# laomao0/BIN

Hardware: AMD Instinct MI355X
Metric: interpolated frames/sec at 1280x720 (higher is better)
Workload: dtype f16x3 (fp16 hi+lo pairs = 22-bit significands, 3 MFMA products, f32 accumulate; fp32-class: 1e-6 vs the fp32 reference); 1 GPU; Adobe240 test_blur 1280x720 inference, batch=1 per GPU (6-frame window padded to 768x1344 by the test.py rule), window-sharded; precision=f16x3, streams=1, pipelined_steps=False, four_call_schedule=False, parity=max-abs <= 2e-5 (f16x3) vs the fp32 reference (tests/)

## Files before the change

### bin_amd/csrc/binhip_conv_x3.hip

```cpp
#include "binhip_conv_common.h"
constexpr int X3_R = 2, X3_WN = 8;

template <int KS, int R, int WN, int NTAP = KS * KS>
struct X3Cfg {
    static constexpr int PAD = KS / 2;
    static constexpr int TH = R * WN;
    static constexpr int PH = TH + KS - 1;
    static constexpr int PW = 32 + KS - 1;
    static constexpr int PP = (PH * PW * 2 + 63) / 64;
    static constexpr int WP = NTAP;
    static constexpr int NW = WN;
    static constexpr int PATCH_BYTES = PP * 1024;
    static constexpr int WBUF_BYTES = 2 * WP * 1024;
    static constexpr int LDS_BYTES = 2 * PATCH_BYTES + 2 * WBUF_BYTES;
    static constexpr int NPJ = (PP + NW - 1) / NW;
    static constexpr int NWJ = (2 * WP + NW - 1) / NW;
    static_assert((KS == 3 ? 2 : 1) * LDS_BYTES <= 160 * 1024, "LDS budget");
};
constexpr int X3_FOLD_TAPS = 20;
template <int KS, int R, int WN, int EPI>
using X3CfgOf = X3Cfg<KS, R, WN, EPI == BINHIP_EPI_SUBPIX_FOLD ? X3_FOLD_TAPS : KS * KS>;

template <class C>
__device__ __forceinline__ void x3_issue_patch(const ConvKArgs& a, char* smem, int c, int pl, int buf, int wave,
                                               const unsigned* voff, const ConvTile& t) {
    __amdgpu_buffer_rsrc_t rs = patch_plane_grouped(a, c, pl, t);
    char* lds = smem + buf * C::PATCH_BYTES;
#pragma unroll
    for (int j = 0; j < C::NPJ; ++j) {
        const int i = wave + C::NW * j;
        if ((C::PP % C::NW == 0) || (i < C::PP))
            __builtin_amdgcn_raw_ptr_buffer_load_lds(rs, (lds_void_t*)(lds + i * 1024), 16, voff[j], 0, 0, 0);
    }
}

template <class C>
__device__ __forceinline__ void x3_issue_weights(const ConvKArgs& a, char* smem, int c, int buf, int wave, int lane, int z) {
    const long long woff = ((long long)z * a.nchunks + c) * (C::WP * 32 * 16);
    __amdgpu_buffer_rsrc_t wh = __builtin_amdgcn_make_buffer_rsrc((void*)(a.w_hi + woff), 0, C::WP * 1024, 0x00020000);
    __amdgpu_buffer_rsrc_t wl = __builtin_amdgcn_make_buffer_rsrc((void*)(a.w_lo + woff), 0, C::WP * 1024, 0x00020000);
    char* lds = smem + 2 * C::PATCH_BYTES + buf * C::WBUF_BYTES;
#pragma unroll
    for (int j = 0; j < C::NWJ; ++j) {
        const int i = wave + C::NW * j;
        if (((2 * C::WP) % C::NW == 0) || (i < 2 * C::WP)) {
            const bool lo = i >= C::WP;
            const int t = lo ? i - C::WP : i;
            __builtin_amdgcn_raw_ptr_buffer_load_lds(lo ? wl : wh, (lds_void_t*)(lds + i * 1024), 16,
                                                     (unsigned)(lane * 16), t * 1024, 0, 0);
        }
    }
}

template <class C, int KS, int R, bool HI>
__device__ __forceinline__ void x3_compute(const char* pb, const char* wb, int a_lane_off, int b_lane_off, floatx16 (&acc)[R]) {
    constexpr int NTAP = KS * KS;
    half8 B[2][R + KS - 1];
    half8 Ah[2], Al[2];
    auto load_b = [&](int dx, half8 (&dst)[R + KS - 1]) {
#pragma unroll
        for (int rr = 0; rr < R + KS - 1; ++rr) dst[rr] = ld8(pb + b_lane_off + (rr * C::PW + dx) * 16);
    };
    auto load_a = [&](int s, half8& h, half8& l) {
        const int dx = s / KS, dy = s % KS;
        const int off = ((dy * KS + dx) * 32) * 32 + a_lane_off;
        h = ld8(wb + off);
        if constexpr (HI) l = ld8(wb + C::WP * 1024 + off);
    };
    load_b(0, B[0]);
    load_a(0, Ah[0], Al[0]);
#pragma unroll
    for (int s = 0; s < NTAP; ++s) {
        const int dx = s / KS, dy = s % KS;
        if (s + 1 < NTAP) load_a(s + 1, Ah[(s + 1) & 1], Al[(s + 1) & 1]);
        if (dy == 0 && dx + 1 < KS) load_b(dx + 1, B[(dx + 1) & 1]);
        __builtin_amdgcn_sched_barrier(0);
        if constexpr (HI) {
#pragma unroll
            for (int r = 0; r < R; ++r)
                acc[r] = mfma_32x32x16(Al[s & 1], B[dx & 1][r + dy], acc[r]);
        }
#pragma unroll
        for (int r = 0; r < R; ++r)
            acc[r] = mfma_32x32x16(Ah[s & 1], B[dx & 1][r + dy], acc[r]);
        __builtin_amdgcn_sched_barrier(0);
    }
}

template <class C, bool HI>
__device__ __forceinline__ void x3_compute_fold(const char* pb, const char* wb, int a_lane_off, int b_lane_off, floatx16& acc) {
    constexpr int NT = 5, NB = 4;
    static_assert(C::WP == NT * NB && C::PH >= 2 * (C::NW - 1) + NT && C::PW >= 32 + NB - 1, "slab and patch of the folded walk");
    half8 B[2][NT];
    half8 Ah[2], Al[2];
    auto load_b = [&](int b, half8 (&dst)[NT]) {
#pragma unroll
        for (int t = 0; t < NT; ++t) dst[t] = ld8(pb + b_lane_off + (t * C::PW + b) * 16);
    };
    auto load_a = [&](int s, half8& h, half8& l) {
        const int b = s / NT, t = s % NT;
        const int off = (t * NB + b) * 1024 + a_lane_off;
        h = ld8(wb + off);
        if constexpr (HI) l = ld8(wb + C::WP * 1024 + off);
    };
    load_b(0, B[0]);
    load_a(0, Ah[0], Al[0]);
#pragma unroll
    for (int s = 0; s < NT * NB; ++s) {
        const int b = s / NT, t = s % NT;
        if (s + 1 < NT * NB) load_a(s + 1, Ah[(s + 1) & 1], Al[(s + 1) & 1]);
        if (t == 0 && b + 1 < NB) load_b(b + 1, B[(b + 1) & 1]);
        __builtin_amdgcn_sched_barrier(0);
        if constexpr (HI) acc = mfma_32x32x16(Al[s & 1], B[b & 1][t], acc);
        acc = mfma_32x32x16(Ah[s & 1], B[b & 1][t], acc);
        __builtin_amdgcn_sched_barrier(0);
    }
}

template <class C, int KS, int R, bool HI>
__device__ __forceinline__ void x3_compute_pair(const char* pb, const char* wb, int n, int kg, int wave, floatx16 (&acc)[R]) {
    static_assert(KS & 1, "odd kernels");
    constexpr int NP = KS / 2;
    const int s16 = ((n >> 3) & 1) << 4;
    const int a_pair = n * 32 + s16 + kg * (KS * 1024);
    const int a_plain = n * 32 + ((kg << 4) ^ s16);
    const int b_pair = ((wave * R + kg) * C::PW + n) * 16;
    const int b_plain = patch_lane_off<C>(n, kg, wave * R);
    half8 Bp[2][R + KS - 3], Bl[2][R];
    half8 Ah[2], Al[2];
    auto load_b = [&](int dx, half8 (&bp)[R + KS - 3], half8 (&bl)[R]) {
#pragma unroll
        for (int rr = 0; rr < R + KS - 3; ++rr) bp[rr] = ld8(pb + b_pair + (rr * C::PW + dx) * 16);
#pragma unroll
        for (int r = 0; r < R; ++r) bl[r] = ld8(pb + b_plain + ((r + KS - 1) * C::PW + dx) * 16);
    };
    auto load_a = [&](int s, half8& h, half8& l) {
        const int dx = s / (NP + 1), j = s % (NP + 1);
        const int off = (j < NP) ? ((2 * j) * KS + dx) * 1024 + a_pair : ((KS - 1) * KS + dx) * 1024 + a_plain;
        h = ld8(wb + off);
        if constexpr (HI) l = ld8(wb + C::WP * 1024 + off);
    };
    constexpr int NS = KS * (NP + 1);
    load_b(0, Bp[0], Bl[0]);
    load_a(0, Ah[0], Al[0]);
#pragma unroll
    for (int s = 0; s < NS; ++s) {
        const int dx = s / (NP + 1), j = s % (NP + 1);
        if (s + 1 < NS) load_a(s + 1, Ah[(s + 1) & 1], Al[(s + 1) & 1]);
        if (j == 0 && dx + 1 < KS) load_b(dx + 1, Bp[(dx + 1) & 1], Bl[(dx + 1) & 1]);
        __builtin_amdgcn_sched_barrier(0);
#pragma unroll
        for (int r = 0; r < R; ++r) {
            const half8 b = (j < NP) ? Bp[dx & 1][r + 2 * j] : Bl[dx & 1][r];
            if constexpr (HI) acc[r] = mfma_32x32x16(Al[s & 1], b, acc[r]);
            acc[r] = mfma_32x32x16(Ah[s & 1], b, acc[r]);
        }
        __builtin_amdgcn_sched_barrier(0);
    }
}

struct X3Gate {
    const unsigned* flags;
    unsigned epoch;
    int chunk;
    unsigned* status;
};
constexpr unsigned RDB3_SPIN_LIMIT = 1u << 22;

template <int KS, int R, int WN, int EPI, bool XTRA, bool GATED = false>
__device__ __forceinline__ void x3_tile(const ConvKArgs& a, const float* __restrict__ bias, char* smem, const ConvTile& t,
                                        const X3Gate gate = X3Gate{nullptr, 0u, 1 << 30, nullptr}) {
    constexpr bool FOLD = EPI == BINHIP_EPI_SUBPIX_FOLD;
    static_assert(!FOLD || (KS == 5 && R == 2 && !XTRA && !GATED), "the folded walk is the 5x5 FINAL_SUBPIX layer's");
    constexpr int RA = FOLD ? 1 : R;
    using C = X3CfgOf<KS, R, WN, EPI>;
    BH_TL_DECL;
    BH_TL_BEGIN();
    const int tid = threadIdx.x;
    const int lane = tid & 63;
    const int wave = __builtin_amdgcn_readfirstlane(tid >> 6);
    const int n = lane & 31;
    const int kg = lane >> 5;
    const int img = t.img, ty = t.ty, tx = t.tx, z = t.z;
    unsigned voff[C::NPJ];
    patch_offsets<C, C::PAD>(voff, t, a.H, a.W, wave, lane);

    floatx16 acc[1][RA];
#pragma unroll
    for (int r = 0; r < RA; ++r)
#pragma unroll
        for (int e = 0; e < 16; ++e) acc[0][r][e] = 0.f;

    const int nchunks = a.nchunks;
    const int a_lane_off = weight_lane_off(n, kg);
    const int b_lane_off = patch_lane_off<C>(n, kg, wave * R);

    __builtin_amdgcn_s_setprio(2);
    x3_issue_weights<C>(a, smem, 0, 0, wave, lane, z);
    if constexpr (GATED) {
        if (gate.chunk <= 0 && gate.flags) {
            if (tid < 9) {
                const int ny = ty + tid / 3 - 1, nx = tx + tid % 3 - 1;
                if (ny >= 0 && ny < a.tiles_y && nx >= 0 && nx < a.tiles_x) {
                    const unsigned* f = gate.flags + ((size_t)img * a.tiles_y + ny) * a.tiles_x + nx;
                    unsigned spins = 0;
                    while (__hip_atomic_load(f, __ATOMIC_RELAXED, __HIP_MEMORY_SCOPE_AGENT) != gate.epoch) {
                        __builtin_amdgcn_s_sleep(2);
                        if (++spins > RDB3_SPIN_LIMIT) {
                            if (gate.status) atomicOr(gate.status, BINHIP_STATUS_SYNC_TIMEOUT);
                            break;
                        }
                    }
                }
            }
            __builtin_amdgcn_s_barrier();
            __builtin_amdgcn_sched_barrier(0);
        }
    }
    x3_issue_patch<C>(a, smem, 0, 0, 0, wave, voff, t);
    for (int c = 0; c < nchunks; ++c) {
        const char* wb = smem + 2 * C::PATCH_BYTES + (c & 1) * C::WBUF_BYTES;
        if (a.prog_prio) {
            const int q = (4 * c) / nchunks;
            if (q == 0) __builtin_amdgcn_s_setprio(3);
            else if (q == 1) __builtin_amdgcn_s_setprio(2);
            else if (q == 2) __builtin_amdgcn_s_setprio(1);
            else __builtin_amdgcn_s_setprio(0);
        }
        wait_vmcnt<0>();
        __builtin_amdgcn_s_barrier();
        __builtin_amdgcn_sched_barrier(0);
#if BINHIP_TIMELINE
        if (c == 0) BH_TL_STAMP(1);
#endif
        x3_issue_patch<C>(a, smem, c, 1, 1, wave, voff, t);
        if (c + 1 < nchunks) x3_issue_weights<C>(a, smem, c + 1, (c + 1) & 1, wave, lane, z);
        unsigned gate_seen = gate.epoch;
        const unsigned* gate_word = nullptr;
        if constexpr (GATED) {
            if (c + 1 == gate.chunk && gate.flags && tid < 9) {
                const int ny = ty + tid / 3 - 1, nx = tx + tid % 3 - 1;
                if (ny >= 0 && ny < a.tiles_y && nx >= 0 && nx < a.tiles_x) {
                    gate_word = gate.flags + ((size_t)img * a.tiles_y + ny) * a.tiles_x + nx;
                    gate_seen = __hip_atomic_load(gate_word, __ATOMIC_RELAXED, __HIP_MEMORY_SCOPE_AGENT);
                }
            }
        }
        const bool pair = (KS == 5) && !XTRA && !FOLD && a.half_last && (c + 1 == nchunks);
        if constexpr (FOLD) {
            x3_compute_fold<C, true>(smem, wb, a_lane_off, b_lane_off, acc[0][0]);
        } else if constexpr (KS == 5 && !XTRA) {
            if (pair) x3_compute_pair<C, KS, R, true>(smem, wb, n, kg, wave, acc[0]);
            else x3_compute<C, KS, R, true>(smem, wb, a_lane_off, b_lane_off, acc[0]);
        } else {
            x3_compute<C, KS, R, true>(smem, wb, a_lane_off, b_lane_off, acc[0]);
        }
        wait_vmcnt<0>();
        __builtin_amdgcn_s_barrier();
        __builtin_amdgcn_sched_barrier(0);
        if constexpr (GATED) {
            if (c + 1 == gate.chunk && gate.flags) {
                if (gate_word) {
                    unsigned spins = 0;
                    while (gate_seen != gate.epoch) {
                        __builtin_amdgcn_s_sleep(2);
                        gate_seen = __hip_atomic_load(gate_word, __ATOMIC_RELAXED, __HIP_MEMORY_SCOPE_AGENT);
                        if (++spins > RDB3_SPIN_LIMIT) {
                            if (gate.status) atomicOr(gate.status, BINHIP_STATUS_SYNC_TIMEOUT);
                            break;
                        }
                    }
                }
                __builtin_amdgcn_s_barrier();
                __builtin_amdgcn_sched_barrier(0);
            }
        }
        if (c + 1 < nchunks) x3_issue_patch<C>(a, smem, c + 1, 0, 0, wave, voff, t);
        if constexpr (FOLD) {
            x3_compute_fold<C, false>(smem + C::PATCH_BYTES, wb, a_lane_off, b_lane_off, acc[0][0]);
        } else if constexpr (KS == 5 && !XTRA) {
            if (pair) x3_compute_pair<C, KS, R, false>(smem + C::PATCH_BYTES, wb, n, kg, wave, acc[0]);
            else x3_compute<C, KS, R, false>(smem + C::PATCH_BYTES, wb, a_lane_off, b_lane_off, acc[0]);
        } else {
            x3_compute<C, KS, R, false>(smem + C::PATCH_BYTES, wb, a_lane_off, b_lane_off, acc[0]);
        }
    }
    BH_TL_STAMP(2);
    __builtin_amdgcn_s_setprio(0);
    if constexpr (FOLD) upnet_fold_epilogue(a, bias, acc[0][0], img, t.ty0 + wave * R, t.tx0, n, kg);
    else conv_epilogue<1, R, 3, EPI, XTRA>(a, bias, acc, img, t.ty0 + wave * R, t.tx0, z * 32, z == 0, n, kg, t.plane_elems);
    BH_TL_FINISH(a, (((img * a.tiles_y + ty) * a.tiles_x + tx) * a.ncol + z));
}

template <int KS, int R, int WN, int EPI, int WIDE, bool XTRA>
__global__ void __launch_bounds__(64 * WN)
    __attribute__((amdgpu_waves_per_eu((KS == 5 && !XTRA) ? WN / 4 : WN / 2, (KS == 5 && !XTRA) ? WN / 4 : WN / 2)))
conv_x3_kernel(const ConvKArgs a, const float* __restrict__ bias) {
    extern __shared__ __attribute__((aligned(16))) char smem[];
    x3_tile<KS, R, WN, EPI, XTRA>(a, bias, smem, tile_decode<X3CfgOf<KS, R, WN, EPI>::TH>(a, a.ncol));
}

struct Rdb3Args {
    ConvKArgs conv[3];
    unsigned* flags;
    unsigned epoch;
    int T;
};

template <int R, int WN>
__global__ void __launch_bounds__(64 * WN) __attribute__((amdgpu_waves_per_eu(WN / 2, WN / 2)))
conv_x3_rdbs_kernel(const Rdb3Args a, const float* __restrict__ bias0, const float* __restrict__ bias1,
                    const float* __restrict__ bias2) {
    extern __shared__ __attribute__((aligned(16))) char smem[];
    const int G = (int)gridDim.x;
    const int b = xcd_band((int)blockIdx.x, G);
#pragma unroll 1
    for (int p = 0; p < 3; ++p) {
        const ConvKArgs& ka = a.conv[p];
        const float* bias = p == 0 ? bias0 : (p == 1 ? bias1 : bias2);
        X3Gate gate;
        gate.flags = p > 0 ? a.flags + (size_t)(p - 1) * a.T : nullptr;
        gate.epoch = a.epoch;
        gate.chunk = ka.nchunks - 2;
        gate.status = ka.flags;
#pragma unroll 1
        for (int t0 = b; t0 < a.T; t0 += G) {
            x3_tile<3, R, WN, BINHIP_EPI_PLANES, false, true>(ka, bias, smem, tile_at<R * WN>(ka, t0, 0), gate);
            asm volatile("s_waitcnt vmcnt(0)" ::: "memory");
            __syncthreads();
            if (threadIdx.x == 0 && p < 2)
                __hip_atomic_store(a.flags + (size_t)p * a.T + t0, a.epoch, __ATOMIC_RELAXED, __HIP_MEMORY_SCOPE_AGENT);
        }
    }
}

template <int KS, int R, int WN, int EPI, int WIDE, bool XTRA>
static int launch_x3_x(const ConvKArgs& ka, int cout_pad, hipStream_t s) {
    using C = X3CfgOf<KS, R, WN, EPI>;
    static std::atomic<unsigned long long> lds_set{0};
    if (int rc = bh_set_max_lds(&conv_x3_kernel<KS, R, WN, EPI, WIDE, XTRA>, C::LDS_BYTES, lds_set)) return rc;
    ConvKArgs a = ka;
    const dim3 grid(set_tiles<C>(a, cout_pad / 32));
    a.prog_prio = (KS == 3 && !XTRA && (long long)grid.x <= 2ll * binhip_device_cus()) ? 1 : 0;
#if BINHIP_TIMELINE
    a.tl = bh_tl_reserve(grid.x, &a.tl_base);
    a.tl_launch = ((KS == 3 && EPI == BINHIP_EPI_PLANES && WIDE == 0 && !XTRA ? 1u : 3u) << 24) | (g_bh_tl_serial.fetch_add(1) & 0xFFFFFFu);
#endif
    conv_x3_kernel<KS, R, WN, EPI, WIDE, XTRA><<<grid, dim3(64 * C::NW), C::LDS_BYTES, s>>>(a, a.bias);
    BH_CHECK_LAUNCH();
    return 0;
}
template <int KS, int R, int WN, int EPI, int WIDE>
static int launch_x3(const ConvKArgs& ka, int cout_pad, hipStream_t s) {
    if constexpr (EPI == BINHIP_EPI_PLANES) {
        if (ka.has_res || ka.r2_hi || ka.m_hi || ka.y_unshuf) return launch_x3_x<KS, R, WN, EPI, WIDE, true>(ka, cout_pad, s);
    }
    return launch_x3_x<KS, R, WN, EPI, WIDE, false>(ka, cout_pad, s);
}

int bh_launch_rdb3_x3(const ConvKArgs* convs, unsigned* flags, unsigned epoch, int cus, hipStream_t s) {
    using C = X3Cfg<3, X3_R, X3_WN>;
    static std::atomic<unsigned long long> lds_set{0};
    static std::atomic<int> per_cu{-1};
    if (int rc = bh_set_max_lds(&conv_x3_rdbs_kernel<X3_R, X3_WN>, C::LDS_BYTES, lds_set)) return rc;
    int occ = per_cu.load(std::memory_order_acquire);
    if (occ < 0) {
        int n = 0;
        hipError_t e = hipOccupancyMaxActiveBlocksPerMultiprocessor(&n, conv_x3_rdbs_kernel<X3_R, X3_WN>, 64 * C::NW,
                                                                    C::LDS_BYTES);
        if (e != hipSuccess) return (int)e;
        occ = n > 2 ? 2 : n;
        per_cu.store(occ, std::memory_order_release);
    }
    if (occ < 1) return BINHIP_E_SHAPE;
    Rdb3Args a;
    for (int p = 0; p < 3; ++p) {
        a.conv[p] = convs[p];
        set_tiles<C>(a.conv[p]);
        if (!a.conv[p].wt || a.conv[p].nchunks < 3) return BINHIP_E_SHAPE;
#if BINHIP_TIMELINE
        a.conv[p].tl = bh_tl_reserve((unsigned)(a.conv[p].tiles_x * a.conv[p].tiles_y * a.conv[p].N), &a.conv[p].tl_base);
        a.conv[p].tl_launch = ((4u + p) << 24) | (g_bh_tl_serial.load() & 0xFFFFFFu);
#endif
    }
#if BINHIP_TIMELINE
    g_bh_tl_serial.fetch_add(1);
#endif
    a.T = a.conv[0].tiles_x * a.conv[0].tiles_y * a.conv[0].N;
    a.flags = flags; a.epoch = epoch;
    const long long slots = (long long)occ * (cus > 0 ? cus : 256);
    const unsigned grid = (unsigned)(a.T < slots ? a.T : slots);
    for (int p = 0; p < 3; ++p) a.conv[p].prog_prio = (a.T <= slots) ? 1 : 0;
    conv_x3_rdbs_kernel<X3_R, X3_WN><<<dim3(grid), dim3(64 * C::NW), C::LDS_BYTES, s>>>(a, a.conv[0].bias, a.conv[1].bias,
                                                                                                   a.conv[2].bias);
    BH_CHECK_LAUNCH();
    return 0;
}

__global__ void __launch_bounds__(256)
final_dot2_kernel(const ConvKArgs a, const unsigned* __restrict__ w_hi32) {
    using C = X3Cfg<3, 2, 4>;
    extern __shared__ __attribute__((aligned(16))) char smem[];
    const int tid = threadIdx.x;
    const int lane = tid & 63;
    const int wave = __builtin_amdgcn_readfirstlane(tid >> 6);
    const ConvTile t = tile_decode<C::TH>(a, 1);
    const int img = t.img, tx0 = t.tx0, ty0 = t.ty0;
    const int H = a.H, W = a.W;
    unsigned voff[C::NPJ];
    patch_offsets<C, C::PAD>(voff, t, H, W, wave, lane);
    const int px = lane & 31, py = 2 * wave + (lane >> 5);
    const int base_off = (py * C::PW + px) * 16;
    float acc[3] = {0.f, 0.f, 0.f};
    typedef _Float16 half2v __attribute__((ext_vector_type(2)));
    union X8 { half8 h; half2v p[4]; };
    union W2 { unsigned u; half2v p; };

    const int nchunks = a.nchunks;
    auto compute = [&](const char* pb, int c) {
        const unsigned* wh = w_hi32 + (long long)c * (9 * 32 * 8);
#pragma unroll
        for (int t = 0; t < 9; ++t) {
            const int dy = t / 3, dx = t % 3;
#pragma unroll
            for (int cg = 0; cg < 2; ++cg) {
                X8 x;
                x.h = *reinterpret_cast<const half8*>(pb + cg * (C::PH * C::PW * 16) + base_off + (dy * C::PW + dx) * 16);
#pragma unroll
                for (int r = 0; r < 3; ++r) {
#pragma unroll
                    for (int k = 0; k < 4; ++k) {
                        W2 w;
                        w.u = wh[(t * 32 + r) * 8 + cg * 4 + k];
                        acc[r] = __builtin_amdgcn_fdot2(x.p[k], w.p, acc[r], false);
                    }
                }
            }
        }
    };

    x3_issue_patch<C>(a, smem, 0, 0, 0, wave, voff, t);
    for (int c = 0; c < nchunks; ++c) {
        wait_vmcnt<0>();
        __builtin_amdgcn_s_barrier();
        __builtin_amdgcn_sched_barrier(0);
        if (c + 1 < nchunks) x3_issue_patch<C>(a, smem, c + 1, 0, (c + 1) & 1, wave, voff, t);
        compute(smem + (c & 1) * C::PATCH_BYTES, c);
    }
    const int gy = ty0 + py, gx = tx0 + px;
    if (gy < H && gx < W) {
        float sum[3], bj[3];
        const int nimg = a.nimg;
#pragma unroll
        for (int j = 0; j < 3; ++j) {
            const long long idx = (((long long)img * a.cout + (j < a.cout ? j : 0)) * H + gy) * W + gx;
            float v[5];
#pragma unroll
            for (int t = 0; t < 5; ++t) v[t] = (t < nimg) ? a.img[t][idx] : 0.f;
            bj[j] = a.bias[j < a.cout ? j : 0];
            float sj = v[0];
#pragma unroll
            for (int t = 1; t < 5; ++t)
                if (t < nimg) sj += v[t];
            sum[j] = nimg > 0 ? sj / (float)nimg : 0.f;
        }
#pragma unroll
        for (int j = 0; j < 3; ++j) asm volatile("" : "+v"(sum[j]), "+v"(bj[j]));
        __builtin_amdgcn_sched_barrier(0);
#pragma unroll
        for (int j = 0; j < 3; ++j) {
            if (j >= a.cout) break;
            const long long idx = (((long long)img * a.cout + j) * H + gy) * W + gx;
            a.out_f32[idx] = (acc[j] + bj[j]) + sum[j];
        }
    }
}

struct M16 {
    using C = X3Cfg<3, 2, 8>;
    static constexpr int NSTAGE = 3;
    static constexpr int WPIECES = 5;
    static constexpr int W_OFF = NSTAGE * C::PATCH_BYTES;
    static constexpr int LDS_BYTES = W_OFF + 2 * WPIECES * 1024;
    static_assert(2 * LDS_BYTES <= 160 * 1024, "two workgroups per CU");
};

template <bool HI>
__device__ __forceinline__ void m16_compute(const char* pb, const char* wb, int a_lane_off, int b_lane_off, int slot, int a_zero,
                                            floatx4 (&acc)[2][2]) {
    using C = X3Cfg<3, 2, 8>;
    half8 Ah[2], Al[2], B[2][2][2];
    auto tap_off = [](int t) { return ((t / 3) * C::PW + (t % 3)) * 16; };
    auto load = [&](int p, half8& ah, half8& al, half8 (&b)[2][2]) {
        const int aoff = (p < 4) ? (2 * p + slot) * 128 + a_lane_off : (slot ? 8 * 128 + a_zero : 8 * 128 + a_lane_off);
        ah = ld8(wb + aoff);
        if constexpr (HI) al = ld8(wb + M16::WPIECES * 1024 + aoff);
        const int boff = b_lane_off + tap_off(2 * p) + slot * (p < 4 ? tap_off(2 * p + 1) - tap_off(2 * p) : 0);
#pragma unroll
        for (int r = 0; r < 2; ++r)
#pragma unroll
            for (int g = 0; g < 2; ++g) b[r][g] = ld8(pb + boff + (r * C::PW + g * 16) * 16);
    };
    load(0, Ah[0], Al[0], B[0]);
#pragma unroll
    for (int p = 0; p < 5; ++p) {
        if (p + 1 < 5) load(p + 1, Ah[(p + 1) & 1], Al[(p + 1) & 1], B[(p + 1) & 1]);
        __builtin_amdgcn_sched_barrier(0);
#pragma unroll
        for (int r = 0; r < 2; ++r)
#pragma unroll
            for (int g = 0; g < 2; ++g) {
                if constexpr (HI) acc[r][g] = __builtin_amdgcn_mfma_f32_16x16x32_f16(Al[p & 1], B[p & 1][r][g], acc[r][g], 0, 0, 0);
                acc[r][g] = __builtin_amdgcn_mfma_f32_16x16x32_f16(Ah[p & 1], B[p & 1][r][g], acc[r][g], 0, 0, 0);
            }
        __builtin_amdgcn_sched_barrier(0);
    }
}

__global__ void __launch_bounds__(512) __attribute__((amdgpu_waves_per_eu(4, 4)))
final_m16_kernel(const ConvKArgs a, const float* __restrict__ bias) {
    using C = X3Cfg<3, 2, 8>;
    extern __shared__ __attribute__((aligned(16))) char smem[];
    const int tid = threadIdx.x;
    const int lane = tid & 63;
    const int wave = __builtin_amdgcn_readfirstlane(tid >> 6);
    const ConvTile t = tile_decode<C::TH>(a, 1);
    const int img = t.img, tx0 = t.tx0, ty0 = t.ty0;
    const int H = a.H, W = a.W;
    unsigned voff[C::NPJ];
    patch_offsets<C, C::PAD>(voff, t, H, W, wave, lane);
    const int n16 = lane & 15, kb = lane >> 4;
    const int slot = kb >> 1;
    const int a_lane_off = ((n16 < 3 ? n16 : 3) * 2 + (kb & 1)) * 16;
    const int a_zero = (3 * 2 + (kb & 1)) * 16;
    const int b_lane_off = ((kb & 1) * (C::PH * C::PW) + wave * 2 * C::PW + n16) * 16;
    floatx4 acc[2][2];
#pragma unroll
    for (int r = 0; r < 2; ++r)
#pragma unroll
        for (int g = 0; g < 2; ++g) acc[r][g] = floatx4{0.f, 0.f, 0.f, 0.f};

    const int nchunks = a.nchunks;
    const int nstage = 2 * nchunks;
    {
        const int ntaps = nchunks * 9;
        for (int i = wave; i < 2 * M16::WPIECES; i += C::NW) {
            const int pl = i >= M16::WPIECES ? 1 : 0;
            const int t = (i - pl * M16::WPIECES) * 8 + (lane >> 3);
            __amdgpu_buffer_rsrc_t rs = __builtin_amdgcn_make_buffer_rsrc((void*)(pl ? a.w_lo : a.w_hi), 0, (unsigned)(ntaps * 1024), 0x00020000);
            const unsigned off = t < ntaps ? (unsigned)(t * 1024 + (lane & 7) * 16) : 0x80000000u;
            __builtin_amdgcn_raw_ptr_buffer_load_lds(rs, (lds_void_t*)(smem + M16::W_OFF + i * 1024), 16, off, 0, 0, 0);
        }
    }
    x3_issue_patch<C>(a, smem, 0, 0, 0, wave, voff, t);
    if (nstage > 1) x3_issue_patch<C>(a, smem, 0, 1, 1, wave, voff, t);
    const bool three = wave < (C::PP - 2 * C::NW);
    for (int s = 0; s < nstage; ++s) {
        if (s + 1 < nstage) {
            if (three) wait_vmcnt<3>(); else wait_vmcnt<2>();
        } else {
            wait_vmcnt<0>();
        }
        __builtin_amdgcn_s_barrier();
        __builtin_amdgcn_sched_barrier(0);
        if (s + 2 < nstage) x3_issue_patch<C>(a, smem, (s + 2) >> 1, (s + 2) & 1, (s + 2) % 3, wave, voff, t);
        const char* pb = smem + (s % 3) * C::PATCH_BYTES;
        const char* wb = smem + M16::W_OFF + (s >> 1) * (9 * 128);
        if (s & 1) m16_compute<false>(pb, wb, a_lane_off, b_lane_off, slot, a_zero, acc);
        else m16_compute<true>(pb, wb, a_lane_off, b_lane_off, slot, a_zero, acc);
    }
    if (kb == 0) {
        float sum[2][2][3];
        const int nimg = a.nimg;
#pragma unroll
        for (int r = 0; r < 2; ++r)
#pragma unroll
            for (int g = 0; g < 2; ++g) {
                const int gy = ty0 + wave * 2 + r, gx = tx0 + g * 16 + n16;
                const bool ok = gy < H && gx < W;
                const int gyc = gy < H ? gy : H - 1, gxc = gx < W ? gx : W - 1;
#pragma unroll
                for (int j = 0; j < 3; ++j) {
                    const long long idx = (((long long)img * a.cout + (j < a.cout ? j : 0)) * H + gyc) * W + gxc;
                    float v[5];
#pragma unroll
                    for (int t = 0; t < 5; ++t) v[t] = (t < nimg) ? a.img[t][idx] : 0.f;
                    float sj = v[0];
#pragma unroll
                    for (int t = 1; t < 5; ++t)
                        if (t < nimg) sj += v[t];
                    sum[r][g][j] = (ok && nimg > 0) ? sj / (float)nimg : 0.f;
                }
            }
        float bj[3];
#pragma unroll
        for (int j = 0; j < 3; ++j) bj[j] = bias[j < a.cout ? j : 0];
#pragma unroll
        for (int r = 0; r < 2; ++r)
#pragma unroll
            for (int g = 0; g < 2; ++g)
#pragma unroll
                for (int j = 0; j < 3; ++j) asm volatile("" : "+v"(sum[r][g][j]));
#pragma unroll
        for (int j = 0; j < 3; ++j) asm volatile("" : "+v"(bj[j]));
        __builtin_amdgcn_sched_barrier(0);
#pragma unroll
        for (int r = 0; r < 2; ++r)
#pragma unroll
            for (int g = 0; g < 2; ++g) {
                const int gy = ty0 + wave * 2 + r, gx = tx0 + g * 16 + n16;
                if (gy >= H || gx >= W) continue;
#pragma unroll
                for (int j = 0; j < 3; ++j) {
                    if (j >= a.cout) break;
                    const long long idx = (((long long)img * a.cout + j) * H + gy) * W + gx;
                    a.out_f32[idx] = (acc[r][g][j] + bj[j]) + sum[r][g][j];
                }
            }
    }
}

int bh_launch_final_m16(const ConvKArgs& ka, hipStream_t s) {
    using C = X3Cfg<3, 2, 8>;
    static std::atomic<unsigned long long> lds_set{0};
    if (ka.nchunks * 9 > M16::WPIECES * 8) return BINHIP_E_SHAPE;
    if (int rc = bh_set_max_lds(&final_m16_kernel, M16::LDS_BYTES, lds_set)) return rc;
    ConvKArgs a = ka;
    final_m16_kernel<<<dim3(set_tiles<C>(a)), dim3(512), M16::LDS_BYTES, s>>>(a, a.bias);
    BH_CHECK_LAUNCH();
    return 0;
}

int bh_launch_final_dot2(const ConvKArgs& ka, hipStream_t s) {
    using C = X3Cfg<3, 2, 4>;
    ConvKArgs a = ka;
    const dim3 grid(set_tiles<C>(a));
    final_dot2_kernel<<<grid, dim3(256), 2 * C::PATCH_BYTES, s>>>(a, reinterpret_cast<const unsigned*>(a.w_hi));
    BH_CHECK_LAUNCH();
    return 0;
}

int bh_launch_conv_x3_k5(const ConvKArgs& a, int cout_pad, hipStream_t s) {
    return launch_x3<5, X3_R, X3_WN, BINHIP_EPI_PLANES, 1>(a, cout_pad, s);
}

int bh_launch_conv_x3_k5_subpix(const ConvKArgs& a, hipStream_t s) {
    if (a.upnet_fold) return launch_x3<5, X3_R, X3_WN, BINHIP_EPI_SUBPIX_FOLD, 0>(a, 32, s);
    return launch_x3<5, X3_R, X3_WN, BINHIP_EPI_FINAL_SUBPIX, 0>(a, 32, s);
}

struct RingArgs {
    const _Float16* x_hi;
    const _Float16* x_lo;
    const float* wvar;
    const float* bvar;
    float* out;
    const float* img[5];
    int N, H, W, cin, nimg;
};
constexpr int RING_THREADS = 128;
__global__ void __launch_bounds__(RING_THREADS) upnet_ring_kernel(const RingArgs a) {
    __shared__ float red[3][RING_THREADS / 64];
    const int tid = threadIdx.x, lane = tid & 63, wave = tid >> 6;
    const int H = a.H, W = a.W, H2 = 2 * H, W2 = 2 * W;
    const int ring = 2 * W2 + 2 * (H2 - 2);
    int id = blockIdx.x;
    const int img = id / ring;
    id -= img * ring;
    int Y, X;
    if (id < W2) { Y = 0; X = id; }
    else if (id < 2 * W2) { Y = H2 - 1; X = id - W2; }
    else { const int k = id - 2 * W2; Y = 1 + (k >> 1); X = (k & 1) ? W2 - 1 : 0; }
    const int y = Y >> 1, i = Y & 1, x = X >> 1, j = X & 1;
    const int vy = (Y == 0) ? 0 : (Y == H2 - 1 ? 2 : 1), vx = (X == 0) ? 0 : (X == W2 - 1 ? 2 : 1);
    const int var = 3 * vy + vx, sub = 2 * i + j;
    const int cin = a.cin, ng = cin >> 3, items = 25 * ng;
    const long long wstride = (long long)25 * cin;
    const float* w = a.wvar + ((long long)var * 12 + sub) * wstride;
    float s0 = 0.f, s1 = 0.f, s2 = 0.f;
    for (int it = tid; it < items; it += RING_THREADS) {
        const int tap = it / ng, ci = (it - tap * ng) << 3;
        const int yy = y + tap / 5 - 2, xx = x + tap % 5 - 2;
        if (yy < 0 || yy >= H || xx < 0 || xx >= W) continue;
        const long long o = (((((long long)(ci >> 4) * a.N + img) * H + yy) * W + xx) << 4) + (ci & 15);
        const half8 xh = *reinterpret_cast<const half8*>(a.x_hi + o);
        half8 xl;
        if (a.x_lo) xl = *reinterpret_cast<const half8*>(a.x_lo + o);
        const float* wq = w + (long long)tap * cin + ci;
        floatx4 wa[3][2];
#pragma unroll
        for (int c = 0; c < 3; ++c) {
            wa[c][0] = *reinterpret_cast<const floatx4*>(wq + 4 * c * wstride);
            wa[c][1] = *reinterpret_cast<const floatx4*>(wq + 4 * c * wstride + 4);
        }
#pragma unroll
        for (int e = 0; e < 8; ++e) {
            float v = (float)xh[e];
            if (a.x_lo) v += (float)xl[e];
            s0 = fmaf(wa[0][e >> 2][e & 3], v, s0);
            s1 = fmaf(wa[1][e >> 2][e & 3], v, s1);
            s2 = fmaf(wa[2][e >> 2][e & 3], v, s2);
        }
    }
#pragma unroll
    for (int off = 32; off > 0; off >>= 1) {
        s0 += __shfl_xor(s0, off);
        s1 += __shfl_xor(s1, off);
        s2 += __shfl_xor(s2, off);
    }
    if (lane == 0) { red[0][wave] = s0; red[1][wave] = s1; red[2][wave] = s2; }
    __syncthreads();
    if (tid < 3) {
        const int c = tid;
        const float v = red[c][0] + red[c][1];
        const long long idx = (((long long)img * 3 + c) * H2 + Y) * W2 + X;
        float m = 0.f;
        if (a.nimg > 0) {
            m = a.img[0][idx];
            for (int t = 1; t < a.nimg; ++t) m += a.img[t][idx];
            m = m / (float)a.nimg;
        }
        a.out[idx] = (v + a.bvar[var * 12 + 4 * c + sub]) + m;
    }
}
int bh_launch_upnet_ring(const void* x_hi, const void* x_lo, const float* wvar, const float* bvar, float* out, const float* const* images,
                         int nimg, int N, int H, int W, int cin, hipStream_t s) {
    if (!x_hi || !wvar || !bvar || !out || N <= 0 || H <= 0 || W <= 0 || cin <= 0 || (cin & 15) || nimg < 0 || nimg > 5) return BINHIP_E_ARG;
    RingArgs a;
    a.x_hi = (const _Float16*)x_hi; a.x_lo = (const _Float16*)x_lo; a.wvar = wvar; a.bvar = bvar; a.out = out;
    for (int t = 0; t < 5; ++t) a.img[t] = (t < nimg) ? images[t] : nullptr;
    a.N = N; a.H = H; a.W = W; a.cin = cin; a.nimg = nimg;
    const long long ring = 4ll * W + 4ll * H - 4;
    upnet_ring_kernel<<<dim3((unsigned)(ring * N)), dim3(RING_THREADS), 0, s>>>(a);
    BH_CHECK_LAUNCH();
    return 0;
}

int bh_launch_conv_x3(const ConvKArgs& a, int cout_pad, int epilogue, hipStream_t s) {
    if (epilogue == BINHIP_EPI_PLANES)
        return cout_pad == 32 ? launch_x3<3, X3_R, X3_WN, BINHIP_EPI_PLANES, 0>(a, cout_pad, s)
                              : launch_x3<3, X3_R, X3_WN, BINHIP_EPI_PLANES, 1>(a, cout_pad, s);
    if (epilogue == BINHIP_EPI_SHUFFLE) return launch_x3<3, X3_R, X3_WN, BINHIP_EPI_SHUFFLE, 1>(a, cout_pad, s);
    if (epilogue == BINHIP_EPI_FINAL) return launch_x3<3, X3_R, X3_WN, BINHIP_EPI_FINAL, 0>(a, cout_pad, s);
    return BINHIP_E_SHAPE;
}
```

Baseline: 16.87 interpolated frames/s.

## Add ring-buffered weight-column pipeline kernel for 5x5 f16x3 convolutions

Adds a new 5x5 conv kernel that streams weights one tap column at a time through a three-slot LDS ring with a prefetch distance of two columns, instead of staging the full KS*KS weight set double-buffered. This shrinks LDS so two workgroups can share a CU and overlaps weight loads with MFMA work at finer granularity. It also adds a paired-row variant for a half-filled last chunk. Plain 5x5 convs without extra epilogue inputs now go to the ring kernel, while others use launch_x3_x. The cost is more barriers per chunk, with one s_barrier per column step.

```diff
diff --git a/bin_amd/csrc/binhip_conv_x3.hip b/bin_amd/csrc/binhip_conv_x3.hip
--- a/bin_amd/csrc/binhip_conv_x3.hip
+++ b/bin_amd/csrc/binhip_conv_x3.hip
@@ -298,6 +298,230 @@
 conv_x3_kernel(const ConvKArgs a, const float* __restrict__ bias) {
     extern __shared__ __attribute__((aligned(16))) char smem[];
     x3_tile<KS, R, WN, EPI, XTRA>(a, bias, smem, tile_decode<X3CfgOf<KS, R, WN, EPI>::TH>(a, a.ncol));
+}
+
+template <int KS, int R, int WN>
+struct X3RingCfg {
+    using C = X3Cfg<KS, R, WN>;
+    static constexpr int NSLOT = 3;
+    static constexpr int NCOL = 2 * KS;
+    static constexpr int COL_PIECES = 2 * KS;
+    static constexpr int SLOT_BYTES = COL_PIECES * 1024;
+    static constexpr int RING_OFF = 2 * C::PATCH_BYTES;
+    static constexpr int LDS_BYTES = RING_OFF + NSLOT * SLOT_BYTES;
+    static constexpr int NCJ = (COL_PIECES + WN - 1) / WN;
+    static_assert(LDS_BYTES <= 80 * 1024, "two workgroups per CU");
+};
+
+__device__ __forceinline__ int x3r_pieces(int n, int wave, int nw) { return wave < n ? (n - wave + nw - 1) / nw : 0; }
+
+__device__ __forceinline__ void wait_vmcnt_upto(int n) {
+    switch (n) {
+        case 0: wait_vmcnt<0>(); break;
+        case 1: wait_vmcnt<1>(); break;
+        case 2: wait_vmcnt<2>(); break;
+        case 3: wait_vmcnt<3>(); break;
+        case 4: wait_vmcnt<4>(); break;
+        default: wait_vmcnt<5>(); break;
+    }
+}
+
+template <class G, int KS, int J>
+__device__ __forceinline__ int x3r_issue_col(const ConvKArgs& a, char* smem, int c, int slot, int wave, int lane, int z) {
+    constexpr int dx = J % KS;
+    constexpr int NP = J < KS ? 2 * KS : KS;
+    const long long woff = ((long long)z * a.nchunks + c) * (KS * KS * 32 * 16);
+    __amdgpu_buffer_rsrc_t wh = __builtin_amdgcn_make_buffer_rsrc((void*)(a.w_hi + woff), 0, KS * KS * 1024, 0x00020000);
+    __amdgpu_buffer_rsrc_t wl = __builtin_amdgcn_make_buffer_rsrc((void*)(a.w_lo + woff), 0, KS * KS * 1024, 0x00020000);
+    char* lds = smem + G::RING_OFF + slot * G::SLOT_BYTES;
+#pragma unroll
+    for (int k = 0; k < G::NCJ; ++k) {
+        const int i = wave + G::C::NW * k;
+        if (i < NP) {
+            const bool lo = i >= KS;
+            const int dy = lo ? i - KS : i;
+            __builtin_amdgcn_raw_ptr_buffer_load_lds(lo ? wl : wh, (lds_void_t*)(lds + i * 1024), 16, (unsigned)(lane * 16),
+                                                     (dy * KS + dx) * 1024, 0, 0);
+        }
+    }
+    return x3r_pieces(NP, wave, G::C::NW);
+}
+
+template <class G, int KS, int R, bool HI, int DX>
+__device__ __forceinline__ void x3r_compute_col(const char* pb, const char* ws, int a_lane_off, int b_lane_off,
+                                                half8 (&B)[2][R + KS - 1], floatx16 (&acc)[R]) {
+    using C = typename G::C;
+    half8 Ah[2], Al[2];
+    auto load_b = [&](int dx, half8 (&dst)[R + KS - 1]) {
+#pragma unroll
+        for (int rr = 0; rr < R + KS - 1; ++rr) dst[rr] = ld8(pb + b_lane_off + (rr * C::PW + dx) * 16);
+    };
+    auto load_a = [&](int dy, half8& h, half8& l) {
+        const int off = dy * 1024 + a_lane_off;
+        h = ld8(ws + off);
+        if constexpr (HI) l = ld8(ws + KS * 1024 + off);
+    };
+    if constexpr (DX == 0) load_b(0, B[0]);
+    load_a(0, Ah[0], Al[0]);
+#pragma unroll
+    for (int dy = 0; dy < KS; ++dy) {
+        if (dy + 1 < KS) load_a(dy + 1, Ah[(dy + 1) & 1], Al[(dy + 1) & 1]);
+        if (dy == 0 && DX + 1 < KS) load_b(DX + 1, B[(DX + 1) & 1]);
+        __builtin_amdgcn_sched_barrier(0);
+        if constexpr (HI) {
+#pragma unroll
+            for (int r = 0; r < R; ++r)
+                acc[r] = mfma_32x32x16(Al[dy & 1], B[DX & 1][r + dy], acc[r]);
+        }
+#pragma unroll
+        for (int r = 0; r < R; ++r)
+            acc[r] = mfma_32x32x16(Ah[dy & 1], B[DX & 1][r + dy], acc[r]);
+        __builtin_amdgcn_sched_barrier(0);
+    }
+}
+
+struct X3RingState {
+    int c, nchunks, slot, after;
+    int wave, lane, z, a_lane_off, b_lane_off;
+};
+
+template <class G, int KS, int R, bool HI, int DX>
+__device__ __forceinline__ void x3r_compute_col_pair(const char* pb, const char* ws, int n, int kg, int wave, half8 (&B)[2][R + KS - 1],
+                                                     floatx16 (&acc)[R]) {
+    using C = typename G::C;
+    static_assert(KS & 1, "odd kernels");
+    constexpr int NP = KS / 2, NPR = R + KS - 3;
+    static_assert(NPR + R <= R + KS - 1, "pair and plain rows share the column's fragment set");
+    const int s16 = ((n >> 3) & 1) << 4;
+    const int a_pair = n * 32 + s16 + kg * 1024;
+    const int a_plain = n * 32 + ((kg << 4) ^ s16) + (KS - 1) * 1024;
+    const int b_pair = ((wave * R + kg) * C::PW + n) * 16;
+    const int b_plain = patch_lane_off<C>(n, kg, wave * R);
+    half8 Ah[2], Al[2];
+    auto load_b = [&](int dx, half8 (&dst)[R + KS - 1]) {
+#pragma unroll
+        for (int rr = 0; rr < NPR; ++rr) dst[rr] = ld8(pb + b_pair + (rr * C::PW + dx) * 16);
+#pragma unroll
+        for (int r = 0; r < R; ++r) dst[NPR + r] = ld8(pb + b_plain + ((r + KS - 1) * C::PW + dx) * 16);
+    };
+    auto load_a = [&](int j, half8& h, half8& l) {
+        const int off = (j < NP) ? (2 * j) * 1024 + a_pair : a_plain;
+        h = ld8(ws + off);
+        if constexpr (HI) l = ld8(ws + KS * 1024 + off);
+    };
+    if constexpr (DX == 0) load_b(0, B[0]);
+    load_a(0, Ah[0], Al[0]);
+#pragma unroll
+    for (int j = 0; j <= NP; ++j) {
+        if (j + 1 <= NP) load_a(j + 1, Ah[(j + 1) & 1], Al[(j + 1) & 1]);
+        if (j == 0 && DX + 1 < KS) load_b(DX + 1, B[(DX + 1) & 1]);
+        __builtin_amdgcn_sched_barrier(0);
+#pragma unroll
+        for (int r = 0; r < R; ++r) {
+            const half8 b = (j < NP) ? B[DX & 1][r + 2 * j] : B[DX & 1][NPR + r];
+            if constexpr (HI) acc[r] = mfma_32x32x16(Al[j & 1], b, acc[r]);
+            acc[r] = mfma_32x32x16(Ah[j & 1], b, acc[r]);
+        }
+        __builtin_amdgcn_sched_barrier(0);
+    }
+}
+
+template <class G, int KS, int R, bool PAIR, int J>
+__device__ __forceinline__ void x3r_step(const ConvKArgs& a, char* smem, const ConvTile& t, const unsigned* voff, X3RingState& st,
+                                         half8 (&B)[2][R + KS - 1], floatx16 (&acc)[R]) {
+    using C = typename G::C;
+    constexpr bool HI = J < KS;
+    wait_vmcnt_upto(st.after);
+    __builtin_amdgcn_s_barrier();
+    __builtin_amdgcn_sched_barrier(0);
+    int wave = st.wave;
+    asm volatile("" : "+s"(wave));
+    int n = 0;
+    if constexpr (J == 0) {
+        x3_issue_patch<C>(a, smem, st.c, 1, 1, wave, voff, t);
+        n += x3r_pieces(C::PP, wave, C::NW);
+    }
+    if constexpr (J == KS) {
+        if (st.c + 1 < st.nchunks) {
+            x3_issue_patch<C>(a, smem, st.c + 1, 0, 0, wave, voff, t);
+            n += x3r_pieces(C::PP, wave, C::NW);
+        }
+    }
+    constexpr int J2 = (J + 2) % G::NCOL;
+    const int c2 = st.c + (J + 2 >= G::NCOL ? 1 : 0);
+    const int slot2 = st.slot >= 1 ? st.slot - 1 : st.slot + 2;
+    if (c2 < st.nchunks) n += x3r_issue_col<G, KS, J2>(a, smem, c2, slot2, wave, st.lane, st.z);
+    st.after = n;
+    const char* ws = smem + G::RING_OFF + st.slot * G::SLOT_BYTES;
+    const char* pb = smem + (HI ? 0 : C::PATCH_BYTES);
+    if constexpr (PAIR) x3r_compute_col_pair<G, KS, R, HI, J % KS>(pb, ws, st.lane & 31, st.lane >> 5, st.wave, B, acc);
+    else x3r_compute_col<G, KS, R, HI, J % KS>(pb, ws, st.a_lane_off, st.b_lane_off, B, acc);
+    st.slot = st.slot == G::NSLOT - 1 ? 0 : st.slot + 1;
+}
+
+template <class G, int KS, int R, bool PAIR, int... Js>
+__device__ __forceinline__ void x3r_chunk(const ConvKArgs& a, char* smem, const ConvTile& t, const unsigned* voff, X3RingState& st,
+                                          half8 (&B)[2][R + KS - 1], floatx16 (&acc)[R], std::integer_sequence<int, Js...>) {
+    (x3r_step<G, KS, R, PAIR, Js>(a, smem, t, voff, st, B, acc), ...);
+}
+
+template <int KS, int R, int WN, bool HALF_LAST>
+__global__ void __launch_bounds__(64 * WN) __attribute__((amdgpu_waves_per_eu(WN / 2, WN / 2)))
+conv_x3_ring_kernel(const ConvKArgs a, const float* __restrict__ bias) {
+    using G = X3RingCfg<KS, R, WN>;
+    using C = typename G::C;
+    static_assert(G::NSLOT == 3 && G::NCOL >= 2, "prefetch distance of two columns");
+    extern __shared__ __attribute__((aligned(16))) char smem[];
+    const ConvTile t = tile_decode<C::TH>(a, a.ncol);
+    BH_TL_DECL;
+    BH_TL_BEGIN();
+    const int tid = threadIdx.x;
+    const int lane = tid & 63;
+    const int wave = __builtin_amdgcn_readfirstlane(tid >> 6);
+    const int n = lane & 31, kg = lane >> 5;
+    unsigned voff[C::NPJ];
+    patch_offsets<C, C::PAD>(voff, t, a.H, a.W, wave, lane);
+    floatx16 acc[1][R];
+#pragma unroll
+    for (int r = 0; r < R; ++r)
+#pragma unroll
+        for (int e = 0; e < 16; ++e) acc[0][r][e] = 0.f;
+    half8 B[2][R + KS - 1];
+    X3RingState st;
+    st.nchunks = a.nchunks; st.wave = wave; st.lane = lane; st.z = t.z; st.slot = 0;
+    st.a_lane_off = weight_lane_off(n, kg);
+    st.b_lane_off = patch_lane_off<C>(n, kg, wave * R);
+
+    __builtin_amdgcn_s_setprio(2);
+    x3_issue_patch<C>(a, smem, 0, 0, 0, wave, voff, t);
+    x3r_issue_col<G, KS, 0>(a, smem, 0, 0, wave, lane, t.z);
+    st.after = x3r_issue_col<G, KS, 1>(a, smem, 0, 1, wave, lane, t.z);
+    BH_TL_STAMP(1);
+    const int nplain = HALF_LAST ? st.nchunks - 1 : st.nchunks;
+    for (st.c = 0; st.c < nplain; ++st.c)
+        x3r_chunk<G, KS, R, false>(a, smem, t, voff, st, B, acc[0], std::make_integer_sequence<int, G::NCOL>{});
+    if constexpr (HALF_LAST) x3r_chunk<G, KS, R, true>(a, smem, t, voff, st, B, acc[0], std::make_integer_sequence<int, G::NCOL>{});
+    BH_TL_STAMP(2);
+    __builtin_amdgcn_s_setprio(0);
+    conv_epilogue<1, R, 3, BINHIP_EPI_PLANES, false>(a, bias, acc, t.img, t.ty0 + wave * R, t.tx0, t.z * 32, t.z == 0, n, kg, t.plane_elems);
+    BH_TL_FINISH(a, (((t.img * a.tiles_y + t.ty) * a.tiles_x + t.tx) * a.ncol + t.z));
+}
+
+template <bool HALF_LAST>
+static int launch_x3_ring(const ConvKArgs& ka, int cout_pad, hipStream_t s) {
+    using G = X3RingCfg<5, X3_R, X3_WN>;
+    static std::atomic<unsigned long long> lds_set{0};
+    if (int rc = bh_set_max_lds(&conv_x3_ring_kernel<5, X3_R, X3_WN, HALF_LAST>, G::LDS_BYTES, lds_set)) return rc;
+    ConvKArgs a = ka;
+    const dim3 grid(set_tiles<G::C>(a, cout_pad / 32));
+    a.prog_prio = 0;
+#if BINHIP_TIMELINE
+    a.tl = bh_tl_reserve(grid.x, &a.tl_base);
+    a.tl_launch = (3u << 24) | (g_bh_tl_serial.fetch_add(1) & 0xFFFFFFu);
+#endif
+    conv_x3_ring_kernel<5, X3_R, X3_WN, HALF_LAST><<<grid, dim3(64 * G::C::NW), G::LDS_BYTES, s>>>(a, a.bias);
+    BH_CHECK_LAUNCH();
+    return 0;
 }
 
 struct Rdb3Args {
@@ -641,7 +865,9 @@
 }
 
 int bh_launch_conv_x3_k5(const ConvKArgs& a, int cout_pad, hipStream_t s) {
-    return launch_x3<5, X3_R, X3_WN, BINHIP_EPI_PLANES, 1>(a, cout_pad, s);
+    const bool xtra = a.has_res || a.r2_hi || a.m_hi || a.y_unshuf;
+    if (!xtra) return a.half_last ? launch_x3_ring<true>(a, cout_pad, s) : launch_x3_ring<false>(a, cout_pad, s);
+    return launch_x3_x<5, X3_R, X3_WN, BINHIP_EPI_PLANES, 1, true>(a, cout_pad, s);
 }
 
 int bh_launch_conv_x3_k5_subpix(const ConvKArgs& a, hipStream_t s) {
```

Measured after the change: 16.93 interpolated frames/s, median of 6. Within noise of the previous version (+0.4%).
